# ml-rust/blazr

Hardware: AMD Instinct MI355X
Metric: decode tokens/sec, Llama-3-8B AWQ-INT4 seq=1 on MI355X (and HBM-roofline fraction) (higher is better)
Workload: dtype i4; 1 GPU; llama3-8b-awq greedy decode, batch 1, seq=1, prompt 16 (seed 26), whole step as one hipGraph; N>1 = independent replicas; resident_weight_bytes=5754585088, context_at_end=242

## Files before the change

blazr_amd/csrc/bz_dev.h:

```cpp
#pragma once
#include "bz_internal.h"
#include <math.h>

typedef unsigned int u32x4_t __attribute__((ext_vector_type(4)));
typedef float f32x4_t __attribute__((ext_vector_type(4)));
__device__ __forceinline__ uint4 ldnt(const uint4* p) {
  const u32x4_t v = __builtin_nontemporal_load((const u32x4_t*)p);
  return make_uint4(v.x, v.y, v.z, v.w);
}
__device__ __forceinline__ float4 ldnt(const float4* p) {
  const f32x4_t v = __builtin_nontemporal_load((const f32x4_t*)p);
  return make_float4(v.x, v.y, v.z, v.w);
}

__device__ __forceinline__ float bf16_round(float x) {
  unsigned u = __float_as_uint(x);
  if ((u & 0x7fffffffu) > 0x7f800000u) return x;
  u += 0x7fffu + ((u >> 16) & 1u);
  return __uint_as_float(u & 0xffff0000u);
}
__device__ __forceinline__ float round_act(float x, int act) {
  if (act == BZ_F16) return f16_round(x);
  if (act == BZ_BF16) return bf16_round(x);
  return x;
}
__device__ __forceinline__ double fix_scale(int act) { return act == BZ_F16 ? 17592186044416.0 : (act == BZ_BF16 ? 1099511627776.0 : 4294967296.0); }
__device__ __forceinline__ double fix_inv(int act) { return act == BZ_F16 ? 5.6843418860808015e-14 : (act == BZ_BF16 ? 9.094947017729282e-13 : 2.3283064365386963e-10); }
__device__ __forceinline__ float fix2f(long long a, int act) {
  const unsigned long long m = a < 0 ? (unsigned long long)(-a) : (unsigned long long)a;
  const double d = fma((double)(unsigned)(m >> 32), 4294967296.0, (double)(unsigned)(m & 0xffffffffull)) * fix_inv(act);
  const float r = (float)d;
  return a < 0 ? -r : r;
}
__device__ __forceinline__ long long f2fix(float p, int act) { return __float2ll_rn(p * (float)fix_scale(act)); }
__device__ __forceinline__ float vsrc_get(const VSrc& s, int i, int act) {
  if (s.fix) return round_act(fix2f(((const long long*)s.p)[i], act), act);
  return ((const float*)s.p)[i];
}
__device__ __forceinline__ float silu_f(float x) { return div_rn(x, 1.0f + bz_expf(-x)); }


#define XQ_NP 8
#define XQ_NM 6
struct OpOr { __device__ __forceinline__ static int f(int a, int b) { return a | b; } };
__device__ __forceinline__ int xq_pack_low(int s6, int s7, int flag) { return (s6 & 0xFFF) | ((s7 & 0xFFF) << 12) | (flag ? (1 << 24) : 0); }
__device__ __forceinline__ bool xq_low(const int4* gpar, int gi) { return __builtin_amdgcn_readfirstlane(gpar[gi + 1].w >> 24) != 0; }

__device__ __forceinline__ void xq_split8(const float (&v)[8], float am, unsigned (&w)[XQ_NP], int (&sp)[XQ_NP], float& cscale) {
  const unsigned eb = (__float_as_uint(am) >> 23) & 255u;
  const bool live = eb >= 32u && eb < 255u;
  const float inv = live ? __uint_as_float((283u - eb) << 23) : 0.f;
  cscale = live ? __uint_as_float((eb - 29u) << 23) : 0.f;
  unsigned code[8];
#pragma unroll
  for (int i = 0; i < 8; i++) code[i] = ((unsigned)(int)rintf(v[i] * inv) + 0x88888888u) ^ 0x88888888u;
  unsigned E[4], O[4];
#pragma unroll
  for (int i = 0; i < 4; i++) {
    E[i] = ((code[i + 4] & 0x0F0F0F0Fu) << 4) | (code[i] & 0x0F0F0F0Fu);
    O[i] = ((code[i] >> 4) & 0x0F0F0F0Fu) | (code[i + 4] & 0xF0F0F0F0u);
  }
#pragma unroll
  for (int k = 0; k < 4; k++) {
    const unsigned sel = 0x0c0c0000u | ((4u + k) << 8) | (unsigned)k;
    const int pe = k == 0 ? 6 : 2 * k - 2, po = k == 0 ? 7 : 2 * k - 1;
    w[pe] = __builtin_amdgcn_perm(E[1], E[0], sel) | (__builtin_amdgcn_perm(E[3], E[2], sel) << 16);
    w[po] = __builtin_amdgcn_perm(O[1], O[0], sel) | (__builtin_amdgcn_perm(O[3], O[2], sel) << 16);
  }
#pragma unroll
  for (int p = 0; p < XQ_NP; p++) sp[p] = __builtin_amdgcn_sdot8((int)w[p], 0x11111111, 0, false);
}
template <int NL>
__device__ __forceinline__ int4 xq_gpar_hi(const unsigned (&w)[XQ_NP], const int (&sp)[XQ_NP]) {
  const int fl = grp_reduce<NL, OpOr>((int)((w[6] | w[7]) != 0u));
  return make_int4(sp[3], sp[4], sp[5], xq_pack_low(sp[6], sp[7], fl));
}

template <int NTH>
__device__ __forceinline__ void quant_x128(const float* xs, int KR, uint4* pl, int4* gpar) {
  unsigned* plw = (unsigned*)pl;
  for (int base = 0; base < KR; base += NTH * 8) {
    const int e0 = base + threadIdx.x * 8;
    const bool on = e0 < KR;
    float v[8];
    if (on) {
      float4 a = *(const float4*)(xs + e0), b = *(const float4*)(xs + e0 + 4);
      v[0] = a.x; v[1] = a.y; v[2] = a.z; v[3] = a.w; v[4] = b.x; v[5] = b.y; v[6] = b.z; v[7] = b.w;
    } else {
#pragma unroll
      for (int i = 0; i < 8; i++) v[i] = 0.f;
    }
    float am = 0.f;
#pragma unroll
    for (int i = 0; i < 8; i++) am = fmaxf(am, fabsf(v[i]));
    am = grp_reduce<16, OpMax>(am);
    unsigned w[XQ_NP]; int sp[XQ_NP]; float cs;
    xq_split8(v, am, w, sp, cs);
#pragma unroll
    for (int p = 0; p < XQ_NP; p++) sp[p] = grp_reduce<16, OpAdd>(sp[p]);
    const int4 g2w = xq_gpar_hi<16>(w, sp);
    if (on) {
      const int word = ((e0 >> 5) * XQ_NP) * 4 + ((e0 >> 3) & 3);
#pragma unroll
      for (int p = 0; p < XQ_NP; p++) plw[word + p * 4] = w[p];
      if ((threadIdx.x & 15) == 0) {
        gpar[2 * (e0 >> 7)] = make_int4(__float_as_int(cs), sp[0], sp[1], sp[2]);
        gpar[2 * (e0 >> 7) + 1] = g2w;
      }
    }
  }
}

__device__ __forceinline__ void quant_x64(const float* a, uint4* pl, int4* gpar) {
  const int t = threadIdx.x;
  if (t >= 64) return;
  const bool on = t < 8;
  float v[8];
#pragma unroll
  for (int i = 0; i < 8; i++) v[i] = on ? a[t * 8 + i] : 0.f;
  float am = 0.f;
#pragma unroll
  for (int i = 0; i < 8; i++) am = fmaxf(am, fabsf(v[i]));
  am = grp_reduce<8, OpMax>(am);
  unsigned w[XQ_NP]; int sp[XQ_NP]; float cs;
  xq_split8(v, am, w, sp, cs);
#pragma unroll
  for (int p = 0; p < XQ_NP; p++) sp[p] = grp_reduce<8, OpAdd>(sp[p]);
  const int4 g2w = xq_gpar_hi<8>(w, sp);
  if (on) {
    unsigned* plw = (unsigned*)pl;
    const int word = ((t >> 2) * XQ_NP) * 4 + (t & 3);
#pragma unroll
    for (int p = 0; p < XQ_NP; p++) plw[word + p * 4] = w[p];
    if (t == 0) {
      gpar[0] = make_int4(__float_as_int(cs), sp[0], sp[1], sp[2]);
      gpar[1] = g2w;
    }
  }
}


__device__ __forceinline__ void q4_chunk(const uint4& w, const uint4* pl8, int (&D)[XQ_NM]) {
  const unsigned W[4] = {w.x, w.y, w.z, w.w};
#pragma unroll
  for (int p = 0; p < XQ_NM; p++) {
    const uint4 P = pl8[p];
    const unsigned X[4] = {P.x, P.y, P.z, P.w};
#pragma unroll
    for (int j = 0; j < 4; j++) D[p] = __builtin_amdgcn_sdot8((int)W[j], (int)X[j], D[p], false);
  }
}
__device__ __forceinline__ void q4_chunk_low(const uint4& w, const uint4* pl8, int (&DL)[2]) {
  const unsigned W[4] = {w.x, w.y, w.z, w.w};
#pragma unroll
  for (int p = 0; p < 2; p++) {
    const uint4 P = pl8[XQ_NM + p];
    const unsigned X[4] = {P.x, P.y, P.z, P.w};
#pragma unroll
    for (int j = 0; j < 4; j++) DL[p] = __builtin_amdgcn_sdot8((int)W[j], (int)X[j], DL[p], false);
  }
}
__device__ __forceinline__ void q4_chunk2(const uint4& wa, const uint4& wb, const uint4* pl8, int (&Da)[XQ_NM], int (&Db)[XQ_NM]) {
  const unsigned Wa[4] = {wa.x, wa.y, wa.z, wa.w}, Wb[4] = {wb.x, wb.y, wb.z, wb.w};
#pragma unroll
  for (int p = 0; p < XQ_NM; p++) {
    const uint4 P = pl8[p];
    const unsigned X[4] = {P.x, P.y, P.z, P.w};
#pragma unroll
    for (int j = 0; j < 4; j++) {
      Da[p] = __builtin_amdgcn_sdot8((int)Wa[j], (int)X[j], Da[p], false);
      Db[p] = __builtin_amdgcn_sdot8((int)Wb[j], (int)X[j], Db[p], false);
    }
  }
}
__device__ __forceinline__ int q4_low(const int (&DL)[2], const int4 g2, int z) {
  const int zz = 8 - z, s6 = (g2.w << 20) >> 20, s7 = (g2.w << 8) >> 20;
  return (DL[0] + zz * s6) + ((DL[1] + zz * s7) << 4);
}
__device__ __forceinline__ double q4_term(const int (&D)[XQ_NM], int lw, const int4 g1, const int4 g2, float s, int z) {
  const int zz = 8 - z;
  const int V0 = D[0] + zz * g1.y, V1 = D[1] + zz * g1.z, V2 = D[2] + zz * g1.w, V3 = D[3] + zz * g2.x, V4 = D[4] + zz * g2.y, V5 = D[5] + zz * g2.z;
  const int lo = V0 + (V1 << 4) + (V2 << 8), hi = V3 + (V4 << 4) + (V5 << 8);
  return (double)(s * __int_as_float(g1.x)) * fma(fma((double)hi, 4096.0, (double)lo), 256.0, (double)lw);
}

template <int OFF, int NCH, int NTOT, bool SB = false>
__device__ __forceinline__ void q4g_consume_at(const uint4 (&w)[NTOT], int co, int gp, const uint4* pl, const int4* gpar, float s, int z, double& y) {
  int D[XQ_NM] = {0, 0, 0, 0, 0, 0};
  if (!xq_low(gpar, gp)) {
#pragma unroll
    for (int c = 0; c < NCH; c++) { q4_chunk(w[OFF + c], pl + (co + c) * XQ_NP, D); if (SB) __builtin_amdgcn_sched_barrier(0); }
    y += q4_term(D, 0, gpar[gp], gpar[gp + 1], s, z);
  } else {
    int DL[2] = {0, 0};
#pragma unroll
    for (int c = 0; c < NCH; c++) { q4_chunk(w[OFF + c], pl + (co + c) * XQ_NP, D); q4_chunk_low(w[OFF + c], pl + (co + c) * XQ_NP, DL); if (SB) __builtin_amdgcn_sched_barrier(0); }
    y += q4_term(D, q4_low(DL, gpar[gp + 1], z), gpar[gp], gpar[gp + 1], s, z);
  }
}
template <int NCH>
__device__ __forceinline__ void q4g_consume_n(const uint4 (&w)[NCH], int co, int gp, const uint4* pl, const int4* gpar, float s, int z, double& y) {
  q4g_consume_at<0, NCH, NCH>(w, co, gp, pl, gpar, s, z, y);
}
__device__ __forceinline__ void q4g_consume(const uint4 (&w)[4], int g, const uint4* pl, const int4* gpar, float s, int z, double& y) {
  q4g_consume_at<0, 4, 4>(w, g * 4, 2 * g, pl, gpar, s, z, y);
}
template <int OA, int OB, bool SB, int NA, int NB>
__device__ __forceinline__ void q4g_consume2_x(const uint4 (&wa)[NA], const uint4 (&wb)[NB], int g, const uint4* pl, const int4* gpar, float sa, int za, float sb, int zb,
                                               double& ya, double& yb) {
  int Da[XQ_NM] = {0, 0, 0, 0, 0, 0}, Db[XQ_NM] = {0, 0, 0, 0, 0, 0};
  const int4 g1 = gpar[2 * g], g2 = gpar[2 * g + 1];
  if (!xq_low(gpar, 2 * g)) {
#pragma unroll
    for (int c = 0; c < 4; c++) { q4_chunk2(wa[OA + c], wb[OB + c], pl + (g * 4 + c) * XQ_NP, Da, Db); if (SB) __builtin_amdgcn_sched_barrier(0); }
    ya += q4_term(Da, 0, g1, g2, sa, za);
    yb += q4_term(Db, 0, g1, g2, sb, zb);
  } else {
    int La[2] = {0, 0}, Lb[2] = {0, 0};
#pragma unroll
    for (int c = 0; c < 4; c++) {
      q4_chunk2(wa[OA + c], wb[OB + c], pl + (g * 4 + c) * XQ_NP, Da, Db);
      q4_chunk_low(wa[OA + c], pl + (g * 4 + c) * XQ_NP, La); q4_chunk_low(wb[OB + c], pl + (g * 4 + c) * XQ_NP, Lb);
      if (SB) __builtin_amdgcn_sched_barrier(0);
    }
    ya += q4_term(Da, q4_low(La, g2, za), g1, g2, sa, za);
    yb += q4_term(Db, q4_low(Lb, g2, zb), g1, g2, sb, zb);
  }
}
template <int OFF, int NTOT>
__device__ __forceinline__ void q4g_consume2_at(const uint4 (&wa)[NTOT], const uint4 (&wb)[NTOT], int g, const uint4* pl, const int4* gpar, float sa, int za, float sb, int zb,
                                                double& ya, double& yb) {
  q4g_consume2_x<OFF, OFF, false>(wa, wb, g, pl, gpar, sa, za, sb, zb, ya, yb);
}
template <int OA, int OB, int NTOT, bool SB = false>
__device__ __forceinline__ void q4g_consume2_ab(const uint4 (&w)[NTOT], int g, const uint4* pl, const int4* gpar, float sa, int za, float sb, int zb, double& ya, double& yb) {
  q4g_consume2_x<OA, OB, SB>(w, w, g, pl, gpar, sa, za, sb, zb, ya, yb);
}

__device__ __forceinline__ long long d2fix(double p, int act) { return __double2ll_rn(p * fix_scale(act)); }

template <int ACT> __device__ __forceinline__ float round_t(float x) {
  if (ACT == BZ_F16) return f16_round(x);
  if (ACT == BZ_BF16) return bf16_round(x);
  return x;
}
#define DPP_ROR4 0x124
#define DPP_ROR8 0x128


__device__ __forceinline__ void lds_wait_count(volatile unsigned* cnt, unsigned n) {
  while (*cnt < n) __builtin_amdgcn_s_sleep(1);
  asm volatile("" ::: "memory");
}

__device__ __forceinline__ size_t kv_row_off(const KvView& kv, int layer, int kvh, int p) {
  if (kv.paged) {
    const int blk = kv.block_table[p / kv.bs];
    return (size_t)layer * kv.layer_stride + (((size_t)blk * kv.n_kv + kvh) * kv.bs + (p % kv.bs)) * kv.hd;
  }
  return (size_t)layer * kv.layer_stride + ((size_t)kvh * kv.cap + p) * kv.hd;
}
__device__ __forceinline__ size_t kv_slot_off(const KvView& kv, int layer, int kvh, int slot) {
  const int blk = slot / kv.bs, o = slot % kv.bs;
  return (size_t)layer * kv.layer_stride + (((size_t)blk * kv.n_kv + kvh) * kv.bs + o) * kv.hd;
}
// ... 38 lines not shown
```

blazr_amd/csrc/bz_kernels.hip:

```cpp
#include "bz_internal.h"
#include "bz_dev.h"
#include "bz_ggml.h"
#include <math.h>

#include <hip/hip_ext.h>

static thread_local BzTimingSink* g_sink = nullptr;
void bzk_set_timing_sink(BzTimingSink* s) { g_sink = s; }
BzTimingSink* bzk_timing_sink() { return g_sink; }

__device__ __forceinline__ float block_sum256(float v, float* red) {
  v = wave_sum(v);
  if ((threadIdx.x & 63) == 0) red[threadIdx.x >> 6] = v;
  __syncthreads();
  float t = (red[0] + red[1]) + (red[2] + red[3]);
  __syncthreads();
  return t;
}

template <int NTH>
__device__ __forceinline__ void zero_duty(long long* zb, int zn) {
  if (zb)
    for (int i = blockIdx.x * NTH + threadIdx.x; i < zn; i += gridDim.x * NTH) zb[i] = 0;
}
// ... 2761 lines not shown
#pragma unroll
    for (int i = 0; i < NV; i++) {
      if (KVDT == BZ_F32) {
        const float4 v = *(const float4*)(src + i * 4);
        raw[i] = make_uint4(__float_as_uint(v.x), __float_as_uint(v.y), __float_as_uint(v.z), __float_as_uint(v.w));
      } else {
        unsigned u[4];
#pragma unroll
        for (int j = 0; j < 4; j++) {
          const float x0 = src[i * 8 + 2 * j], x1 = src[i * 8 + 2 * j + 1];
          if (KVDT == BZ_F16) u[j] = (unsigned)__half_as_ushort(f16_cvt(x0)) | ((unsigned)__half_as_ushort(f16_cvt(x1)) << 16);
          else u[j] = (__float_as_uint(bf16_round(x0)) >> 16) | (__float_as_uint(bf16_round(x1)) & 0xffff0000u);
        }
        raw[i] = make_uint4(u[0], u[1], u[2], u[3]);
      }
    }
  }
  __device__ __forceinline__ float get(int e) const {
    if (KVDT == BZ_F32) {
      const uint4 v = raw[e >> 2];
      const unsigned u = (e & 3) == 0 ? v.x : ((e & 3) == 1 ? v.y : ((e & 3) == 2 ? v.z : v.w));
      return __uint_as_float(u);
    }
    const uint4 v = raw[e >> 3];
    const int w = (e >> 1) & 3;
    const unsigned u = w == 0 ? v.x : (w == 1 ? v.y : (w == 2 ? v.z : v.w));
    if (KVDT == BZ_F16) return __half2float(__ushort_as_half((unsigned short)((e & 1) ? (u >> 16) : (u & 0xffffu))));
    return __uint_as_float((e & 1) ? (u & 0xffff0000u) : (u << 16));
  }
};

template <int HD, int KVDT>
__global__ __launch_bounds__(256) void k_attn_decode(AttnArgs a) {
  extern __shared__ __attribute__((aligned(16))) char smem[];
  constexpr int half = HD / 2;
  constexpr int LDR = HD + 4;
  const int rep = a.nq / a.nkv;
  float* qs = (float*)smem;
  float* knew = qs + HD;
  float* vnew = knew + HD;
  float* wred = vnew + HD;
  float* ored = wred + 8;
  const int hq = blockIdx.x, kvh = hq / rep;
  const int tid = threadIdx.x, wave = __builtin_amdgcn_readfirstlane(tid >> 6), lane = tid & 63;
  const int pos = a.pos[0];
  const int len = a.q_only ? pos : pos + 1;
  const int ncache = pos;
  const KvView& kv = a.kv;
  zero_duty<256>(a.zero_buf, a.zero_n);

  if (!a.q_only) {
    const float* cr = a.cos_t + (size_t)pos * half;
    const float* sr = a.sin_t + (size_t)pos * half;
    for (int idx = tid; idx < 2 * half; idx += 256) {
      const int hh = idx / half, i = idx % half;
      const int base = hh == 0 ? hq * HD : a.nq * HD + kvh * HD;
      const int ia = a.interleaved ? 2 * i : i, ib = a.interleaved ? 2 * i + 1 : i + half;
      const float x0 = vsrc_get(a.qkv, base + ia, a.act), x1 = vsrc_get(a.qkv, base + ib, a.act);
      const float c = cr[i], s = sr[i];
      const float y0 = round_act(rope_lo(x0, x1, c, s), a.act), y1 = round_act(rope_hi(x0, x1, c, s), a.act);
      if (hh == 0) { qs[ia] = y0; qs[ib] = y1; }
      else { knew[ia] = y0; knew[ib] = y1; }
    }
    for (int i = tid; i < HD; i += 256) vnew[i] = vsrc_get(a.qkv, a.nq * HD + a.nkv * HD + kvh * HD + i, a.act);
    __syncthreads();
    if (hq % rep == 0) {
      size_t woff;
      if (kv.paged) woff = kv_slot_off(kv, a.layer, kvh, kv.slot ? kv.slot[0] : (kv.block_table[pos / kv.bs] * kv.bs + pos % kv.bs));
      else woff = kv_row_off(kv, a.layer, kvh, pos);
      for (int i = tid; i < HD; i += 256) { kv_st(kv.k, woff + i, kv.dtype, knew[i]); kv_st(kv.v, woff + i, kv.dtype, vnew[i]); }
    }
  } else {
    for (int i = tid; i < HD; i += 256) qs[i] = ((const float*)a.qkv.p)[hq * HD + i];
    __syncthreads();
  }

  const float scale = div_rn(1.0f, sqrt_rn((float)HD));
  float m = -INFINITY, l = 0.f;
  float o[HD];
#pragma unroll
  for (int i = 0; i < HD; i++) o[i] = 0.f;
  for (int p = tid; p < len; p += 256) {
    KvRow<HD, KVDT> kr, vr;
    const size_t ro = p < ncache ? kv_row_off(kv, a.layer, kvh, p) : 0;
    if (p < ncache) kr.load(kv.k, ro); else kr.from_f32(knew);
    if (KVDT != BZ_F32) { if (p < ncache) vr.load(kv.v, ro); else vr.from_f32(vnew); }
    float d = 0.f;
#pragma unroll
    for (int i = 0; i < HD; i += 4) {
      const float4 qa = *(const float4*)(qs + i);
      d += kr.get(i) * qa.x + kr.get(i + 1) * qa.y + kr.get(i + 2) * qa.z + kr.get(i + 3) * qa.w;
    }
    if (KVDT == BZ_F32) { if (p < ncache) vr.load(kv.v, ro); else vr.from_f32(vnew); }
    const float s = d * scale;
    if (m == -INFINITY) {
      m = s; l = 1.f;
#pragma unroll
      for (int i = 0; i < HD; i++) o[i] = vr.get(i);
    } else {
      const float mn = fmaxf(m, s);
      const float alpha = bz_expf(m - mn), e = bz_expf(s - mn);
      l = l * alpha + e;
      m = mn;
#pragma unroll
      for (int i = 0; i < HD; i++) o[i] = o[i] * alpha + e * vr.get(i);
    }
  }
  const float wm = wave_max(m);
  if (lane == 0) wred[wave] = wm;
  __syncthreads();
  const float M = fmaxf(fmaxf(wred[0], wred[1]), fmaxf(wred[2], wred[3]));
  const float w = (m == -INFINITY) ? 0.f : bz_expf(m - M);
  const float ws = wave_sum(l * w);
  if (lane == 0) wred[4 + wave] = ws;
  const int nrows = min(len, 256);
  if (tid < nrows) {
#pragma unroll
    for (int i = 0; i < HD; i += 4) *(float4*)(ored + tid * LDR + i) = make_float4(o[i] * w, o[i + 1] * w, o[i + 2] * w, o[i + 3] * w);
  }
  __syncthreads();
  const float inv = div_rn(1.0f, (wred[4] + wred[5]) + (wred[6] + wred[7]));
  constexpr int PH = 256 / HD;
  const int col = tid % HD, ph = tid / HD;
  float acc = 0.f;
  for (int r = ph; r < nrows; r += PH) acc += ored[r * LDR + col];
  __syncthreads();
  ored[ph * LDR + col] = acc;
  __syncthreads();
  if (tid < HD) {
    float t = 0.f;
#pragma unroll
    for (int q = 0; q < PH; q++) t += ored[q * LDR + tid];
    a.out[(size_t)hq * HD + tid] = round_act(t * inv, a.act);
  }
}


template <int KVDT, int FUSE, int TPW, int NW, int PAGED, int HD = 128>
__global__ __launch_bounds__(NW * 64) void k_attn2(AttnArgs a, const uint4* __restrict__ W, const __half* __restrict__ S,
                                               const unsigned char* __restrict__ Z, const float* __restrict__ bias, int CS, long long* acc) {
  static_assert(HD == 128 || (HD == 64 && FUSE != 1), "head_dim 128, or 64 without the int4 o_proj");
  constexpr int half = HD / 2, NPC = HD / 8, RPL = 64 / NPC, PW = 256 / NW, NL = PW / RPL, OW = NW > 8 ? 8 : NW, NTH = NW * 64;
  asm volatile("" :: "s"(a.zero_buf), "s"(a.zero_n), "s"(a.kv.k), "s"(a.kv.v), "s"(a.kv.cap), "s"(a.kv.layer_stride), "s"(a.layer), "s"(a.act),
               "s"(a.interleaved), "s"(a.rope_cur), "s"(a.qkv.p), "s"(a.qkv.fix), "s"(a.nq), "s"(a.nkv), "s"(a.q_only), "s"(a.pos), "s"(W), "s"(S),
               "s"(Z), "s"(bias), "s"(CS), "s"(acc), "s"(a.out), "s"(a.kv.bs), "s"(a.kv.n_kv));
  extern __shared__ __attribute__((aligned(16))) char smem[];
  unsigned* q2 = (unsigned*)smem;
  unsigned* k2 = q2 + 64;
  unsigned* v2 = k2 + 64;
  double* pout = (double*)(v2 + 64);
  double* lred = pout + NW * 128;
  float* wred = (float*)(lred + NW);
  float* outh = wred + 2 * NW;
  uint4* xpl = (uint4*)(outh + 128);
  int4* gpar = (int4*)(xpl + 4 * XQ_NP);
  const int rep = a.nq / a.nkv;
  const int hq = FUSE ? blockIdx.x / CS : blockIdx.x, cs = FUSE ? blockIdx.x % CS : 0, kvh = hq / rep;
  const int tid = threadIdx.x, wave = __builtin_amdgcn_readfirstlane(tid >> 6), lane = tid & 63;
  const int piece = lane % NPC, rsub = lane / NPC;
  const KvView& kv = a.kv;
  const int pos_v = a.pos[0];
  const int slot_v = PAGED ? *(kv.slot ? kv.slot : a.pos) : 0;
  const int fixq = a.q_only ? 0 : a.qkv.fix;
  int i0, i1;
  {
    const int hh = tid / half, i = tid % half;
    const int base = hh == 0 ? hq * HD : a.nq * HD + kvh * HD;
    const int ia = a.interleaved ? 2 * i : i, ib = a.interleaved ? 2 * i + 1 : i + half;
    const int vb = a.nq * HD + a.nkv * HD + kvh * HD + 2 * i;
    i0 = hh < 2 ? base + ia : vb; i1 = hh < 2 ? base + ib : vb + 1;
    if (a.q_only) { i0 = hq * HD + 2 * i; i1 = i0 + 1; }
    if (hh > 2) { i0 = 0; i1 = 0; }
  }
  unsigned r0l, r0h, r1l, r1h;
  vsrc_issue(a.qkv.p, fixq, i0, r0l, r0h);
  vsrc_issue(a.qkv.p, fixq, i1, r1l, r1h);
  const float* rc = a.q_only ? (const float*)a.qkv.p : a.rope_cur;
  const float pc = rc[tid % half], ps = rc[half + tid % half];
  if (a.zero_buf) {
    const int nblk = FUSE ? a.nq * CS : a.nq;
    for (int i = blockIdx.x * NTH + tid; i < a.zero_n; i += nblk * NTH) a.zero_buf[i] = 0;
  }
  uint4 Wb[FUSE == 1 ? TPW : 1][4];
  const int t0 = (cs * OW + wave % OW) * TPW;
  constexpr int DLD = FUSE == 2 ? TPW : 1;
  uint4 Wd[DLD];
  const int nd0 = (cs * NW + wave) * DLD * RPL;
  if (FUSE == 2) {
    const int K = a.nq * HD;
    const unsigned short* wd = (const unsigned short*)W;
#pragma unroll
    for (int t = 0; t < DLD; t++) Wd[t] = ldnt((const uint4*)(wd + (size_t)(nd0 + t * RPL + rsub) * K + hq * HD + piece * 8));
  }
  if (FUSE == 1) {
    const int K = a.nq * HD;
#pragma unroll
    for (int t = 0; t < TPW; t++) {
      const uint4* wp = W + ((size_t)(t0 + t) * (K >> 5) + hq * 4) * 64 + lane;
#pragma unroll
      for (int c = 0; c < 4; c++) Wb[t][c] = ldnt(wp + c * 64);
    }
  }
  __builtin_amdgcn_sched_barrier(0);
  const int pos = __builtin_amdgcn_readfirstlane(pos_v);
  const int pmax = pos > 0 ? pos - 1 : 0;
  const int len = a.q_only ? pos : pos + 1;
  const unsigned short* kb0 = (const unsigned short*)kv.k + (size_t)a.layer * kv.layer_stride;
  const unsigned short* vb0 = (const unsigned short*)kv.v + (size_t)a.layer * kv.layer_stride;
  uint4 kr[NL], vr[NL];
#pragma unroll
  for (int i = 0; i < NL; i++) { kr[i] = make_uint4(0, 0, 0, 0); vr[i] = make_uint4(0, 0, 0, 0); }
#define ATT_ROW(i) (((i) * NW + wave) * RPL + rsub)
#define ATT_LIVE(c0_, i) ((c0_) + ((i) * NW + wave) * RPL < len)
  if (wave * RPL < len) {
    if (!PAGED) {
      const unsigned short* kb = kb0 + (size_t)kvh * kv.cap * HD;
      const unsigned short* vb = vb0 + (size_t)kvh * kv.cap * HD;
#pragma unroll
      for (int i = 0; i < NL; i++) {
        if (ATT_LIVE(0, i)) {
          const unsigned off = (unsigned)min(ATT_ROW(i), pmax) * HD + piece * 8;
          kr[i] = *(const uint4*)(kb + off);
          vr[i] = *(const uint4*)(vb + off);
        }
      }
    } else {
      int blk[NL];
#pragma unroll
      for (int i = 0; i < NL; i++) blk[i] = ATT_LIVE(0, i) ? kv.block_table[min(ATT_ROW(i), pmax) / kv.bs] : 0;
#pragma unroll
      for (int i = 0; i < NL; i++) {
        if (ATT_LIVE(0, i)) {
          const int pp = min(ATT_ROW(i), pmax);
          const size_t off = (((size_t)blk[i] * kv.n_kv + kvh) * kv.bs + (pp % kv.bs)) * HD + piece * 8;
          kr[i] = *(const uint4*)(kb0 + off);
          vr[i] = *(const uint4*)(vb0 + off);
        }
      }
    }
  }
  const float px0 = vsrc_finish(fixq, r0l, r0h, a.act), px1 = vsrc_finish(fixq, r1l, r1h, a.act);
  if (!a.q_only) {
    if (tid < 2 * half) {
      const int hh = tid / half, i = tid % half;
      const int ia = a.interleaved ? 2 * i : i, ib = a.interleaved ? 2 * i + 1 : i + half;
      const float y0 = round_act(rope_lo(px0, px1, pc, ps), a.act), y1 = round_act(rope_hi(px0, px1, pc, ps), a.act);
      unsigned short* dst = (unsigned short*)(hh == 0 ? q2 : k2);
      const unsigned p0 = pack2<KVDT>(y0, y1);
      dst[ia] = (unsigned short)(p0 & 0xffffu);
      dst[ib] = (unsigned short)(p0 >> 16);
    } else if (tid < 3 * half) {
      v2[tid - 2 * half] = pack2<KVDT>(px0, px1);
    }
    __syncthreads();
    if (hq % rep == 0 && cs == 0 && tid < half) {
      size_t woff;
      if (PAGED) woff = kv_slot_off(kv, a.layer, kvh, kv.slot ? slot_v : (kv.block_table[pos / kv.bs] * kv.bs + pos % kv.bs));
      else woff = kv_row_off_t<0>(kv, a.layer, kvh, pos);
      ((unsigned*)((unsigned short*)kv.k + woff))[tid] = k2[tid];
      ((unsigned*)((unsigned short*)kv.v + woff))[tid] = v2[tid];
    }
  } else {
    if (tid < half) q2[tid] = pack2<KVDT>(px0, px1);
    __syncthreads();
  }

  const float scale = div_rn(1.0f, sqrt_rn((float)HD));
  const uint4 qq = ((const uint4*)q2)[piece];
  float qf[8];
  unpack2<KVDT>(qq.x, qf[0], qf[1]); unpack2<KVDT>(qq.y, qf[2], qf[3]); unpack2<KVDT>(qq.z, qf[4], qf[5]); unpack2<KVDT>(qq.w, qf[6], qf[7]);
  const bool single = len <= 256;
  float sc_[NL];
  float Mw = -INFINITY;
#define ATT_SCORES(c0_)                                                                                                    \
  _Pragma("unroll") for (int i = 0; i < NL; i++) {                                                                         \
    if (!ATT_LIVE(c0_, i)) { sc_[i] = -INFINITY; continue; }                                                               \
    const int p = (c0_) + ATT_ROW(i);                                                                                      \
    uint4 kk = kr[i];                                                                                                      \
    if (!a.q_only && p == pos) { kk = ((const uint4*)k2)[piece]; vr[i] = ((const uint4*)v2)[piece]; }                      \
    float kf[8];                                                                                                           \
    unpack2<KVDT>(kk.x, kf[0], kf[1]); unpack2<KVDT>(kk.y, kf[2], kf[3]); unpack2<KVDT>(kk.z, kf[4], kf[5]); unpack2<KVDT>(kk.w, kf[6], kf[7]); \
    double d = 0.0;                                                                                                        \
    _Pragma("unroll") for (int e = 0; e < 8; e++) d = fma((double)kf[e], (double)qf[e], d);                                \
    d = grp_sum_d<NPC>(d);                                                                                                 \
    sc_[i] = (p < len) ? (float)d * scale : -INFINITY;                                                                     \
  }
  for (int c0 = 0; c0 < len; c0 += 256) {
    const bool won = c0 + wave * RPL < len;
    if (!won) continue;
    if (c0 > 0) {
#pragma unroll
      for (int i = 0; i < NL; i++)
        if (ATT_LIVE(c0, i)) kr[i] = *(const uint4*)(kb0 + kv_row_off_t<PAGED>(kv, 0, kvh, min(c0 + ATT_ROW(i), pmax)) + piece * 8);
    }
    ATT_SCORES(c0)
#pragma unroll
    for (int i = 0; i < NL; i++) Mw = fmaxf(Mw, sc_[i]);
  }
  Mw = wave_max(Mw);
  if (lane == 0) wred[wave] = Mw;
  __syncthreads();
  float Mall = wred[0];
#pragma unroll
  for (int w = 1; w < NW; w++) Mall = fmaxf(Mall, wred[w]);
  double accv[8] = {0.0, 0.0, 0.0, 0.0, 0.0, 0.0, 0.0, 0.0};
  double lsum = 0.0;
  for (int c0 = 0; c0 < len; c0 += 256) {
    const bool won = c0 + wave * RPL < len;
    if (!won) continue;
    if (!single) {
#pragma unroll
      for (int i = 0; i < NL; i++) {
        if (ATT_LIVE(c0, i)) {
          const size_t off = kv_row_off_t<PAGED>(kv, 0, kvh, min(c0 + ATT_ROW(i), pmax)) + piece * 8;
          kr[i] = *(const uint4*)(kb0 + off);
          vr[i] = *(const uint4*)(vb0 + off);
        }
      }
      ATT_SCORES(c0)
    }
#pragma unroll
    for (int i = 0; i < NL; i++) {
      if (!ATT_LIVE(c0, i)) continue;
      const float e = (sc_[i] == -INFINITY) ? 0.f : bz_expf(sc_[i] - Mall);
      const double ed = (double)e;
      lsum += ed;
      float v[8];
      unpack2<KVDT>(vr[i].x, v[0], v[1]); unpack2<KVDT>(vr[i].y, v[2], v[3]);
      unpack2<KVDT>(vr[i].z, v[4], v[5]); unpack2<KVDT>(vr[i].w, v[6], v[7]);
#pragma unroll
      for (int q = 0; q < 8; q++) accv[q] = fma(ed, (double)v[q], accv[q]);
    }
  }
#undef ATT_SCORES
#undef ATT_LIVE
#undef ATT_ROW
  if (NPC == 8) lsum += dpp_get<DPP_ROR8>(lsum);
  lsum = xrow32_d(xrow16_d(lsum));
#pragma unroll
  for (int q = 0; q < 8; q++) {
    if (NPC == 8) accv[q] += dpp_get<DPP_ROR8>(accv[q]);
    accv[q] = xrow32_d(xrow16_d(accv[q]));
  }
  if (lane < NPC) {
#pragma unroll
    for (int q = 0; q < 8; q++) pout[wave * HD + piece * 8 + q] = accv[q];
  }
  if (lane == 0) lred[wave] = lsum;
  __syncthreads();
  float Orun = 0.f, Lrun = 1.f;
  if (tid < HD) {
    double oc = 0.0, Lc = 0.0;
#pragma unroll
    for (int w = 0; w < NW; w++) { oc += pout[w * HD + tid]; Lc += lred[w]; }
    Orun = (float)oc; Lrun = (float)Lc;
  }
  if (!FUSE) {
    if (tid < HD) a.out[(size_t)hq * HD + tid] = round_act(div_rn(Orun, Lrun), a.act);
    return;
  }
  if (tid < HD) outh[tid] = round_act(div_rn(Orun, Lrun), a.act);
  if (FUSE == 2) {
    __syncthreads();
    const float4 oa = *(const float4*)(outh + piece * 8), ob = *(const float4*)(outh + piece * 8 + 4);
    const float of8[8] = {oa.x, oa.y, oa.z, oa.w, ob.x, ob.y, ob.z, ob.w};
#pragma unroll
    for (int t = 0; t < DLD; t++) {
      float w8[8];
      unpack2<KVDT>(Wd[t].x, w8[0], w8[1]); unpack2<KVDT>(Wd[t].y, w8[2], w8[3]); unpack2<KVDT>(Wd[t].z, w8[4], w8[5]); unpack2<KVDT>(Wd[t].w, w8[6], w8[7]);
      double d = 0.0;
#pragma unroll
      for (int e = 0; e < 8; e++) d += (double)__fmul_rn(w8[e], of8[e]);
      d = grp_sum_d<NPC>(d);
      const int n = nd0 + t * RPL + rsub;
      if (piece == 0) {
        if (bias != nullptr && hq == 0) d += (double)bias[n];
        atomicAdd((unsigned long long*)(acc + n), (unsigned long long)d2fix(d, a.act));
      }
    }
    return;
  }
  float sc[FUSE == 1 ? TPW : 1]; int zp[FUSE == 1 ? TPW : 1];
  {
    const int G = (a.nq * HD) >> 7;
#pragma unroll
    for (int t = 0; t < (FUSE == 1 ? TPW : 1); t++) {
      sc[t] = __half2float(S[((size_t)(t0 + t) * G + hq) * 64 + lane]);
      zp[t] = Z[((size_t)(t0 + t) * G + hq) * 64 + lane];
    }
  }
  __syncthreads();
  quant_x128<NW * 64>(outh, HD, xpl, gpar);
  __syncthreads();
#pragma unroll
  for (int t = 0; t < (FUSE == 1 ? TPW : 1); t++) {
    double y = 0.0;
    q4g_consume(Wb[t], 0, xpl, gpar, sc[t], zp[t], y);
    const int n = (t0 + t) * 64 + lane;
    if (bias != nullptr && hq == 0) y += (double)bias[n];
    if (wave < OW) atomicAdd((unsigned long long*)(acc + n), (unsigned long long)d2fix(y, a.act));
  }
}


template <int PAGED, int FUSE = 0>
__global__ __launch_bounds__(512) void k_attn2f(AttnArgs a, const uint4* __restrict__ Wq, const uint4* __restrict__ Hd, const float* __restrict__ bias, int CS, long long* acc) {
  constexpr int HD = 128, half = 64, NW = 8, PW = 256 / NW, NL = PW / 4, NTH = NW * 64;
  __shared__ __attribute__((aligned(16))) float qf[HD], kf[HD], vf[HD];
  __shared__ float wred[2 * NW];
  __shared__ __attribute__((aligned(16))) float pout[NW * 128];
  __shared__ __attribute__((aligned(16))) float outh[FUSE ? HD : 4];
  __shared__ __attribute__((aligned(16))) unsigned xh[FUSE ? 32 : 4], xm[FUSE ? 32 : 4], xl[FUSE ? 32 : 4];
  __shared__ int4 cpar[FUSE ? 8 : 1];
  asm volatile("" :: "s"(a.zero_buf), "s"(a.zero_n), "s"(a.kv.k), "s"(a.kv.v), "s"(a.kv.cap), "s"(a.kv.layer_stride), "s"(a.layer), "s"(a.act),
               "s"(a.interleaved), "s"(a.rope_cur), "s"(a.qkv.p), "s"(a.qkv.fix), "s"(a.nq), "s"(a.nkv), "s"(a.q_only), "s"(a.pos), "s"(a.out),
               "s"(a.kv.bs), "s"(a.kv.n_kv), "s"(Wq), "s"(Hd), "s"(bias), "s"(CS), "s"(acc));
  const int rep = a.nq / a.nkv;
  const int hq = FUSE ? blockIdx.x / CS : blockIdx.x, cs = FUSE ? blockIdx.x % CS : 0, kvh = hq / rep;
  const int tid = threadIdx.x, wave = __builtin_amdgcn_readfirstlane(tid >> 6), lane = tid & 63;
  const int piece = lane & 15, rsub = lane >> 4;
  const KvView& kv = a.kv;
  const int pos_v = a.pos[0];
  const int slot_v = PAGED ? *(kv.slot ? kv.slot : a.pos) : 0;
  const int fixq = a.q_only ? 0 : a.qkv.fix;
  int i0, i1;
  {
    const int hh = tid / half, i = tid % half;
    const int base = hh == 0 ? hq * HD : a.nq * HD + kvh * HD;
    const int ia = a.interleaved ? 2 * i : i, ib = a.interleaved ? 2 * i + 1 : i + half;
    const int vb = a.nq * HD + a.nkv * HD + kvh * HD + 2 * i;
    i0 = hh < 2 ? base + ia : vb; i1 = hh < 2 ? base + ib : vb + 1;
    if (a.q_only) { i0 = hq * HD + 2 * i; i1 = i0 + 1; }
    if (hh > 2) { i0 = 0; i1 = 0; }
  }
  unsigned r0l, r0h, r1l, r1h;
  vsrc_issue(a.qkv.p, fixq, i0, r0l, r0h);
  vsrc_issue(a.qkv.p, fixq, i1, r1l, r1h);
  const float* rc = a.q_only ? (const float*)a.qkv.p : a.rope_cur;
  const float pc = rc[tid % half], ps = rc[half + tid % half];
  if (a.zero_buf)
    for (int i = blockIdx.x * NTH + tid; i < a.zero_n; i += (FUSE ? a.nq * CS : a.nq) * NTH) a.zero_buf[i] = 0;
  uint4 Wb[4]; uint4 hdw = make_uint4(0, 0, 0, 0);
  const int t0 = cs * NW + wave;
  if (FUSE) {
    const int K = a.nq * HD;
    const uint4* wp = Wq + ((size_t)t0 * (K >> 5) + hq * 4) * 64 + lane;
#pragma unroll
    for (int c = 0; c < 4; c++) Wb[c] = ldnt(wp + c * 64);
    hdw = Hd[((size_t)t0 * (K >> 8) + (hq >> 1)) * 64 + lane];
  }
  __builtin_amdgcn_sched_barrier(0);
  const int pos = __builtin_amdgcn_readfirstlane(pos_v);
  const int pmax = pos > 0 ? pos - 1 : 0;
  const int len = a.q_only ? pos : pos + 1;
  const float* kb0 = (const float*)kv.k + (size_t)a.layer * kv.layer_stride;
  const float* vb0 = (const float*)kv.v + (size_t)a.layer * kv.layer_stride;
  float4 kr[NL][2], vr[NL][2];
#pragma unroll
  for (int i = 0; i < NL; i++) { kr[i][0] = kr[i][1] = vr[i][0] = vr[i][1] = make_float4(0.f, 0.f, 0.f, 0.f); }
#define ATF_ROW(i) (((i) * NW + wave) * 4 + rsub)
#define ATF_LIVE(c0_, i) ((c0_) + ((i) * NW + wave) * 4 < len)
  if (wave * 4 < len) {
#pragma unroll
    for (int i = 0; i < NL; i++) {
      if (ATF_LIVE(0, i)) {
        const size_t off = kv_row_off_t<PAGED>(kv, 0, kvh, min(ATF_ROW(i), pmax)) + piece * 8;
        kr[i][0] = *(const float4*)(kb0 + off); kr[i][1] = *(const float4*)(kb0 + off + 4);
        vr[i][0] = *(const float4*)(vb0 + off); vr[i][1] = *(const float4*)(vb0 + off + 4);
      }
    }
  }
  const float px0 = vsrc_finish(fixq, r0l, r0h, a.act), px1 = vsrc_finish(fixq, r1l, r1h, a.act);
  if (!a.q_only) {
    if (tid < 2 * half) {
      const int hh = tid / half, i = tid % half;
      const int ia = a.interleaved ? 2 * i : i, ib = a.interleaved ? 2 * i + 1 : i + half;
      float* dst = hh == 0 ? qf : kf;
      dst[ia] = round_act(rope_lo(px0, px1, pc, ps), a.act);
      dst[ib] = round_act(rope_hi(px0, px1, pc, ps), a.act);
    } else if (tid < 2 * half + 64) {
      vf[2 * (tid - 2 * half)] = px0; vf[2 * (tid - 2 * half) + 1] = px1;
    }
    __syncthreads();
    if (hq % rep == 0 && cs == 0 && tid < HD) {
      size_t woff;
      if (PAGED) woff = kv_slot_off(kv, a.layer, kvh, kv.slot ? slot_v : (kv.block_table[pos / kv.bs] * kv.bs + pos % kv.bs));
      else woff = kv_row_off_t<0>(kv, a.layer, kvh, pos);
      ((float*)kv.k)[woff + tid] = kf[tid];
      ((float*)kv.v)[woff + tid] = vf[tid];
    }
  } else {
    if (tid < 64) { qf[2 * tid] = px0; qf[2 * tid + 1] = px1; }
    __syncthreads();
  }
  const float scale = div_rn(1.0f, sqrt_rn((float)HD));
  const float4 qa = *(const float4*)(qf + piece * 8), qb = *(const float4*)(qf + piece * 8 + 4);
  float Mrun = -INFINITY, Lrun = 0.f, Orun = 0.f;
  for (int c0 = 0; c0 < len; c0 += 256) {
    const bool won = c0 + wave * 4 < len;
    if (c0 > 0) {
      __syncthreads();
      if (won) {
#pragma unroll
        for (int i = 0; i < NL; i++) {
          if (ATF_LIVE(c0, i)) {
            const size_t off = kv_row_off_t<PAGED>(kv, 0, kvh, min(c0 + ATF_ROW(i), pmax)) + piece * 8;
            kr[i][0] = *(const float4*)(kb0 + off); kr[i][1] = *(const float4*)(kb0 + off + 4);
            vr[i][0] = *(const float4*)(vb0 + off); vr[i][1] = *(const float4*)(vb0 + off + 4);
          }
        }
      }
    }
    float sc_[NL];
    float mloc = -INFINITY;
    if (won) {
#pragma unroll
      for (int i = 0; i < NL; i++) {
        if (!ATF_LIVE(c0, i)) { sc_[i] = -INFINITY; continue; }
        const int p = c0 + ATF_ROW(i);
        float4 k0 = kr[i][0], k1 = kr[i][1];
        if (!a.q_only && p == pos) {
          k0 = *(const float4*)(kf + piece * 8); k1 = *(const float4*)(kf + piece * 8 + 4);
          vr[i][0] = *(const float4*)(vf + piece * 8); vr[i][1] = *(const float4*)(vf + piece * 8 + 4);
        }
        float d = k0.x * qa.x + k0.y * qa.y + k0.z * qa.z + k0.w * qa.w + k1.x * qb.x + k1.y * qb.y + k1.z * qb.z + k1.w * qb.w;
        d = grp_reduce<16, OpAdd>(d);
        sc_[i] = (p < len) ? d * scale : -INFINITY;
        mloc = fmaxf(mloc, sc_[i]);
      }
      mloc = wave_max(mloc);
    }
    if (lane == 0) wred[wave] = mloc;
    __syncthreads();
    float Mc = wred[0];
#pragma unroll
    for (int w = 1; w < NW; w++) Mc = fmaxf(Mc, wred[w]);
    float accv[8] = {0.f, 0.f, 0.f, 0.f, 0.f, 0.f, 0.f, 0.f};
    float lsum = 0.f;
    if (won) {
#pragma unroll
      for (int i = 0; i < NL; i++) {
        if (!ATF_LIVE(c0, i)) continue;
        const float e = (sc_[i] == -INFINITY) ? 0.f : bz_expf(sc_[i] - Mc);
        lsum += e;
        accv[0] = fmaf(e, vr[i][0].x, accv[0]); accv[1] = fmaf(e, vr[i][0].y, accv[1]); accv[2] = fmaf(e, vr[i][0].z, accv[2]); accv[3] = fmaf(e, vr[i][0].w, accv[3]);
        accv[4] = fmaf(e, vr[i][1].x, accv[4]); accv[5] = fmaf(e, vr[i][1].y, accv[5]); accv[6] = fmaf(e, vr[i][1].z, accv[6]); accv[7] = fmaf(e, vr[i][1].w, accv[7]);
      }
      lsum = xrow32<OpAdd>(xrow16<OpAdd>(lsum));
#pragma unroll
      for (int q = 0; q < 8; q++) accv[q] = xrow32<OpAdd>(xrow16<OpAdd>(accv[q]));
    }
    if (lane < 16) {
      *(float4*)(pout + wave * 128 + piece * 8) = make_float4(accv[0], accv[1], accv[2], accv[3]);
      *(float4*)(pout + wave * 128 + piece * 8 + 4) = make_float4(accv[4], accv[5], accv[6], accv[7]);
    }
    if (lane == 0) wred[NW + wave] = lsum;
    __syncthreads();
    if (tid < 128) {
      float oc = 0.f, Lc = 0.f;
#pragma unroll
      for (int w = 0; w < NW; w += 2) { oc += pout[w * 128 + tid] + pout[(w + 1) * 128 + tid]; Lc += wred[NW + w] + wred[NW + w + 1]; }
      const float Mn = fmaxf(Mrun, Mc);
      const float fa = (Mrun == -INFINITY) ? 0.f : bz_expf(Mrun - Mn), fb = bz_expf(Mc - Mn);
      Orun = Orun * fa + oc * fb;
      Lrun = Lrun * fa + Lc * fb;
      Mrun = Mn;
    }
  }
  if (!FUSE) {
    if (tid < 128) a.out[(size_t)hq * HD + tid] = round_act(div_rn(Orun, Lrun), a.act);
    return;
  }
  if (tid < 128) outh[tid] = round_act(div_rn(Orun, Lrun), a.act);
  __syncthreads();
  quant_x32<GQ_Q4K>(outh, HD, xh, xm, xl, cpar);
  __syncthreads();
  {
    const unsigned hw[4] = {hdw.x, hdw.y, hdw.z, hdw.w};
    const float d = __half2float(__ushort_as_half((unsigned short)(hw[0] & 0xffffu)));
    const float dmin = __half2float(__ushort_as_half((unsigned short)(hw[0] >> 16)));
    float y = 0.f;
    if (hq & 1) {
#pragma unroll
      for (int c = 0; c < 4; c++) y += gq_chunk_q4k(Wb[c], c, 4 + c, hw, d, dmin, (const uint4*)xh, (const uint4*)xm, (const uint4*)xl, cpar);
    } else {
#pragma unroll
      for (int c = 0; c < 4; c++) y += gq_chunk_q4k(Wb[c], c, c, hw, d, dmin, (const uint4*)xh, (const uint4*)xm, (const uint4*)xl, cpar);
    }
    const int n = t0 * 64 + lane;
    if (bias != nullptr && hq == 0) y += bias[n];
    atomicAdd((unsigned long long*)(acc + n), (unsigned long long)f2fix(y, a.act));
  }
}

static size_t attn2_smem(int nw) { return (size_t)(64 * 3 + 2 * nw + 128 + 4 * XQ_NP * 4 + 8) * 4 + (size_t)(nw * 128 + nw) * 8; }

static int attn_oproj_plan(const AttnArgs& a, const LinearDev& L, int& NW) {
  NW = 0;
  if (a.hd != 128 || L.kind != LK_Q4G || L.perm != nullptr || L.K != a.nq * 128 || a.q_only) return 0;
  const int NT = L.N / 64;
  for (int nw = 8; nw >= 4; nw >>= 1) {
    const int ow = nw > 8 ? 8 : nw;
    for (int cs = 8; cs >= 1; cs >>= 1)
      if (NT % (cs * ow) == 0 && NT / (cs * ow) <= 2 && a.nq * cs <= 1024) { NW = nw; return cs; }
  }
  return 0;
}
static int attn2f_oproj_slices(const AttnArgs& a, const LinearDev& L) {
  static const bool off = getenv("BZ_NO_ATTN_F32") != nullptr;
  if (off || a.hd != 128 || a.kv.dtype != BZ_F32 || a.rope_cur == nullptr || a.q_only || L.kind != LK_Q4K || L.K != a.nq * 128 || L.N % 512 || L.K % 256) return 0;
  const int cs = L.N / 512;
  return a.nq * cs <= 2048 ? cs : 0;
}
static int attn_dense_oproj_loads(const AttnArgs& a, const LinearDev& L) {
  static const bool off = getenv("BZ_NO_ATTN2_HD64") != nullptr;
  if (off || L.kind != LK_ROWS || L.wdt != a.kv.dtype || (a.kv.dtype != BZ_F16 && a.kv.dtype != BZ_BF16) || (a.hd != 64 && a.hd != 128) || a.q_only || a.rope_cur == nullptr) return 0;
  if (L.K != a.nq * a.hd || a.nq * 8 > 2048) return 0;
  const int rpl = 512 / a.hd, per_wave = L.N / 64;
  if (L.N % 64 || per_wave % rpl) return 0;
  const int loads = per_wave / rpl;
  return (loads == 1 || loads == 2 || loads == 4) ? loads : 0;
}
int bzk_attn_oproj_slices(const AttnArgs& a, const LinearDev& L) {
  if (a.kv.dtype == BZ_F32) return attn2f_oproj_slices(a, L);
  if (L.kind == LK_ROWS) return attn_dense_oproj_loads(a, L) > 0 ? 8 : 0;
  int nw; return attn_oproj_plan(a, L, nw);
}

int bzk_attn_oproj(hipStream_t s, const AttnArgs& a, const LinearDev& L, long long* acc) {
  if (a.kv.dtype == BZ_F32) {
    const int CS = attn2f_oproj_slices(a, L);
    if (CS <= 0) BZ_FAIL(BZ_E_INVALID, "attn+o_proj fusion (f32 cache) does not apply to this shape");
    if (a.kv.paged) BZ_LAUNCH("attn+o_proj<q4_K>", L.algo_bytes, (k_attn2f<1, 1>), dim3(a.nq * CS), dim3(512), 0, s, a, (const uint4*)L.w, (const uint4*)L.hdr, L.bias, CS, acc);
    else BZ_LAUNCH("attn+o_proj<q4_K>", L.algo_bytes, (k_attn2f<0, 1>), dim3(a.nq * CS), dim3(512), 0, s, a, (const uint4*)L.w, (const uint4*)L.hdr, L.bias, CS, acc);
    BZ_HIP(hipGetLastError());
    return BZ_OK;
  }
  if (L.kind == LK_ROWS) {
    const int DL = attn_dense_oproj_loads(a, L);
    if (DL <= 0) BZ_FAIL(BZ_E_INVALID, "attn+o_proj fusion (dense) does not apply to this shape");
#define LAUNCH_AD(DT, T, PG, HDV) BZ_LAUNCH("attn+o_proj<dense>", L.algo_bytes, (k_attn2<DT, 2, T, 8, PG, HDV>), dim3(a.nq * 8), dim3(512), attn2_smem(8), s, a, \
    (const uint4*)L.w, (const __half*)nullptr, (const unsigned char*)nullptr, L.bias, 8, acc)
#define LAUNCH_AD_P(DT, T, HDV) do { if (a.kv.paged) LAUNCH_AD(DT, T, 1, HDV); else LAUNCH_AD(DT, T, 0, HDV); } while (0)
#define LAUNCH_AD_T(DT, HDV) do { if (DL == 1) LAUNCH_AD_P(DT, 1, HDV); else if (DL == 2) LAUNCH_AD_P(DT, 2, HDV); else LAUNCH_AD_P(DT, 4, HDV); } while (0)
#define LAUNCH_AD_H(DT) do { if (a.hd == 64) LAUNCH_AD_T(DT, 64); else LAUNCH_AD_T(DT, 128); } while (0)
    if (a.kv.dtype == BZ_F16) LAUNCH_AD_H(BZ_F16); else LAUNCH_AD_H(BZ_BF16);
#undef LAUNCH_AD_H
#undef LAUNCH_AD_T
#undef LAUNCH_AD_P
#undef LAUNCH_AD
    BZ_HIP(hipGetLastError());
    return BZ_OK;
  }
  int NW;
  const int CS = attn_oproj_plan(a, L, NW);
  if (CS <= 0) BZ_FAIL(BZ_E_INVALID, "attn+o_proj fusion does not apply to this shape");
  const int TPW = (L.N / 64) / (CS * (NW > 8 ? 8 : NW));
#define LAUNCH_AO(DT, T, W_, PG) BZ_LAUNCH("attn+o_proj", L.algo_bytes, (k_attn2<DT, 1, T, W_, PG>), dim3(a.nq * CS), dim3(W_ * 64), attn2_smem(W_), s, a, \
    (const uint4*)L.w, (const __half*)L.scales, (const unsigned char*)L.zeros, L.bias, CS, acc)
#define LAUNCH_AO_W(DT, T, PG) do { if (NW == 8) LAUNCH_AO(DT, T, 8, PG); else LAUNCH_AO(DT, T, 4, PG); } while (0)
#define LAUNCH_AO_P(DT, T) do { if (a.kv.paged) LAUNCH_AO_W(DT, T, 1); else LAUNCH_AO_W(DT, T, 0); } while (0)
#define LAUNCH_AO_T(DT) do { if (TPW == 1) LAUNCH_AO_P(DT, 1); else LAUNCH_AO_P(DT, 2); } while (0)
  if (a.kv.dtype == BZ_F16) LAUNCH_AO_T(BZ_F16);
  else if (a.kv.dtype == BZ_BF16) LAUNCH_AO_T(BZ_BF16);
  else BZ_FAIL(BZ_E_UNSUPPORTED, "attn+o_proj fusion: f32 KV cache not built");
#undef LAUNCH_AO_P
#undef LAUNCH_AO_W
#undef LAUNCH_AO_T
#undef LAUNCH_AO
  BZ_HIP(hipGetLastError());
  return BZ_OK;
}


#define ATT_PSTRIDE 132
#define ATT_MAX_SPLITS 128

__host__ __device__ __forceinline__ int att_split_len(int len) {
  int spl = 128;
  while ((len + spl - 1) / spl > ATT_MAX_SPLITS) spl *= 2;
  return spl;
}

template <int KVDT, int PAGED, int REP>
__global__ __launch_bounds__(REP == 8 ? 512 : 256) void k_attn_split(AttnArgs a, int nsplit, float* __restrict__ ws) {
  constexpr int HD = 128, half = 64, NW = REP == 8 ? 8 : 4, NTH = NW * 64, PW = 128 / NW, NL = PW / 4;
  __shared__ __attribute__((aligned(16))) unsigned q2[REP][64];
  __shared__ __attribute__((aligned(16))) unsigned k2[64], v2[64];
  __shared__ float wred[REP][NW], lred[REP][NW];
  __shared__ __attribute__((aligned(16))) float pout[NW][REP][128];
  asm volatile("" :: "s"(a.kv.k), "s"(a.kv.v), "s"(a.kv.cap), "s"(a.kv.layer_stride), "s"(a.layer), "s"(a.act), "s"(a.interleaved), "s"(a.rope_cur),
               "s"(a.qkv.p), "s"(a.qkv.fix), "s"(a.nq), "s"(a.nkv), "s"(a.pos), "s"(nsplit), "s"(ws), "s"(a.kv.bs), "s"(a.kv.n_kv),
               "s"(a.zero_buf), "s"(a.zero_n));
  const int kvh = blockIdx.x / nsplit, s = blockIdx.x % nsplit;
  const int tid = threadIdx.x, wave = __builtin_amdgcn_readfirstlane(tid >> 6), lane = tid & 63;
  const int piece = lane & 15, rsub = lane >> 4;
  const KvView& kv = a.kv;
  const int pos_v = a.pos[0];
  const int slot_v = PAGED ? *(kv.slot ? kv.slot : a.pos) : 0;
  const int hl = min(tid / half, REP - 1), i = tid % half;
  const int ia = a.interleaved ? 2 * i : i, ib = a.interleaved ? 2 * i + 1 : i + half;
  const int qb = (kvh * REP + hl) * HD;
  unsigned q0l, q0h, q1l, q1h, n0l, n0h, n1l, n1h;
  vsrc_issue(a.qkv.p, a.qkv.fix, qb + ia, q0l, q0h);
  vsrc_issue(a.qkv.p, a.qkv.fix, qb + ib, q1l, q1h);
  {
    const int kb_ = a.nq * HD + kvh * HD, vb_ = a.nq * HD + a.nkv * HD + kvh * HD;
    const bool isk = tid < half;
    vsrc_issue(a.qkv.p, a.qkv.fix, isk ? kb_ + ia : vb_ + 2 * i, n0l, n0h);
    vsrc_issue(a.qkv.p, a.qkv.fix, isk ? kb_ + ib : vb_ + 2 * i + 1, n1l, n1h);
  }
  const float pc = a.rope_cur[i], ps = a.rope_cur[half + i];
  if (a.zero_buf)
    for (int z = blockIdx.x * NTH + tid; z < a.zero_n; z += gridDim.x * NTH) a.zero_buf[z] = 0;
  const int pos = __builtin_amdgcn_readfirstlane(pos_v);
  const int len = pos + 1, pmax = pos > 0 ? pos - 1 : 0;
  const int SPL = att_split_len(len);
  const int p0 = s * SPL;
  if (p0 >= len) return;
  const int p1 = min(p0 + SPL, len);
  const bool owner = p1 == len;
  {
    const float x0 = vsrc_finish(a.qkv.fix, q0l, q0h, a.act), x1 = vsrc_finish(a.qkv.fix, q1l, q1h, a.act);
    const unsigned pk = pack2<KVDT>(round_act(rope_lo(x0, x1, pc, ps), a.act), round_act(rope_hi(x0, x1, pc, ps), a.act));
    ((unsigned short*)q2[hl])[ia] = (unsigned short)(pk & 0xffffu);
    ((unsigned short*)q2[hl])[ib] = (unsigned short)(pk >> 16);
  }
  if (owner && tid < 2 * half) {
    const float x0 = vsrc_finish(a.qkv.fix, n0l, n0h, a.act), x1 = vsrc_finish(a.qkv.fix, n1l, n1h, a.act);
    if (tid < half) {
      const unsigned pk = pack2<KVDT>(round_act(rope_lo(x0, x1, pc, ps), a.act), round_act(rope_hi(x0, x1, pc, ps), a.act));
      ((unsigned short*)k2)[ia] = (unsigned short)(pk & 0xffffu);
      ((unsigned short*)k2)[ib] = (unsigned short)(pk >> 16);
    } else {
      v2[i] = pack2<KVDT>(x0, x1);
    }
  }
  __syncthreads();
  if (owner && tid < 64) {
    size_t woff;
    if (PAGED) woff = kv_slot_off(kv, a.layer, kvh, kv.slot ? slot_v : (kv.block_table[pos / kv.bs] * kv.bs + pos % kv.bs));
    else woff = kv_row_off_t<0>(kv, a.layer, kvh, pos);
    ((unsigned*)((unsigned short*)kv.k + woff))[tid] = k2[tid];
    ((unsigned*)((unsigned short*)kv.v + woff))[tid] = v2[tid];
  }
  const unsigned short* kb0 = (const unsigned short*)kv.k + (size_t)a.layer * kv.layer_stride;
  const unsigned short* vb0 = (const unsigned short*)kv.v + (size_t)a.layer * kv.layer_stride;
  const float scale = div_rn(1.0f, sqrt_rn((float)HD));
// ... 1797 lines not shown
```

Baseline: 679.2 tokens/s.

## Make fused attention o_proj tail per-wave to drop block barriers

In the fused attention plus int4 o_proj kernel, each wave now redundantly combines the partial attention outputs, normalizes them, and quantizes the head vector into its own LDS slice. Only wave-level fences are used, replacing the two block-wide __syncthreads around a shared quantization. The AWQ scale and zero-point loads are hoisted next to the weight prefetch so their latency overlaps the attention work. The cost is more LDS per block and duplicated reduction and quantization work in every wave, which could lower occupancy.

```diff
diff --git a/blazr_amd/csrc/bz_dev.h b/blazr_amd/csrc/bz_dev.h
--- a/blazr_amd/csrc/bz_dev.h
+++ b/blazr_amd/csrc/bz_dev.h
@@ -111,6 +111,36 @@
   }
 }
 
+__device__ __forceinline__ void quant_x128_wave(const float* xs, uint4* pl, int4* gpar, int lane) {
+  const int e0 = (lane & 15) * 8;
+  const float4 a = *(const float4*)(xs + e0), b = *(const float4*)(xs + e0 + 4);
+  const float v[8] = {a.x, a.y, a.z, a.w, b.x, b.y, b.z, b.w};
+  float am = 0.f;
+#pragma unroll
+  for (int i = 0; i < 8; i++) am = fmaxf(am, fabsf(v[i]));
+  am = grp_reduce<16, OpMax>(am);
+  unsigned w[XQ_NP]; int sp[XQ_NP]; float cs;
+  xq_split8(v, am, w, sp, cs);
+#pragma unroll
+  for (int p = 0; p < XQ_NP; p++) sp[p] = grp_reduce<16, OpAdd>(sp[p]);
+  const int4 g2w = xq_gpar_hi<16>(w, sp);
+  if (lane < 16) {
+    unsigned* plw = (unsigned*)pl;
+    const int word = ((e0 >> 5) * XQ_NP) * 4 + ((e0 >> 3) & 3);
+#pragma unroll
+    for (int p = 0; p < XQ_NP; p++) plw[word + p * 4] = w[p];
+    if (lane == 0) {
+      gpar[0] = make_int4(__float_as_int(cs), sp[0], sp[1], sp[2]);
+      gpar[1] = g2w;
+    }
+  }
+}
+__device__ __forceinline__ void wave_lds_sync() {
+  __builtin_amdgcn_fence(__ATOMIC_RELEASE, "wavefront");
+  __builtin_amdgcn_wave_barrier();
+  __builtin_amdgcn_fence(__ATOMIC_ACQUIRE, "wavefront");
+}
+
 __device__ __forceinline__ void quant_x64(const float* a, uint4* pl, int4* gpar) {
   const int t = threadIdx.x;
   if (t >= 64) return;
diff --git a/blazr_amd/csrc/bz_kernels.hip b/blazr_amd/csrc/bz_kernels.hip
--- a/blazr_amd/csrc/bz_kernels.hip
+++ b/blazr_amd/csrc/bz_kernels.hip
@@ -2937,8 +2937,8 @@
   double* lred = pout + NW * 128;
   float* wred = (float*)(lred + NW);
   float* outh = wred + 2 * NW;
-  uint4* xpl = (uint4*)(outh + 128);
-  int4* gpar = (int4*)(xpl + 4 * XQ_NP);
+  uint4* xpl = (uint4*)(outh + NW * 128);
+  int4* gpar = (int4*)(xpl + NW * 4 * XQ_NP);
   const int rep = a.nq / a.nkv;
   const int hq = FUSE ? blockIdx.x / CS : blockIdx.x, cs = FUSE ? blockIdx.x % CS : 0, kvh = hq / rep;
   const int tid = threadIdx.x, wave = __builtin_amdgcn_readfirstlane(tid >> 6), lane = tid & 63;
@@ -2977,6 +2977,7 @@
 #pragma unroll
     for (int t = 0; t < DLD; t++) Wd[t] = ldnt((const uint4*)(wd + (size_t)(nd0 + t * RPL + rsub) * K + hq * HD + piece * 8));
   }
+  unsigned short sraw[FUSE == 1 ? TPW : 1]; int zp[FUSE == 1 ? TPW : 1];
   if (FUSE == 1) {
     const int K = a.nq * HD;
 #pragma unroll
@@ -2984,6 +2985,12 @@
       const uint4* wp = W + ((size_t)(t0 + t) * (K >> 5) + hq * 4) * 64 + lane;
 #pragma unroll
       for (int c = 0; c < 4; c++) Wb[t][c] = ldnt(wp + c * 64);
+    }
+    const int G = K >> 7;
+#pragma unroll
+    for (int t = 0; t < TPW; t++) {
+      sraw[t] = ((const unsigned short*)S)[((size_t)(t0 + t) * G + hq) * 64 + lane];
+      zp[t] = Z[((size_t)(t0 + t) * G + hq) * 64 + lane];
     }
   }
   __builtin_amdgcn_sched_barrier(0);
@@ -3133,6 +3140,31 @@
   }
   if (lane == 0) lred[wave] = lsum;
   __syncthreads();
+  if constexpr (FUSE == 1) {
+    float* oh = outh + wave * HD;
+    uint4* xw = xpl + wave * 4 * XQ_NP;
+    int4* gw = gpar + wave * 2;
+    double o0 = 0.0, o1 = 0.0, Lc = 0.0;
+#pragma unroll
+    for (int w = 0; w < NW; w++) {
+      const double2 pp = *(const double2*)(pout + w * HD + 2 * lane);
+      o0 += pp.x; o1 += pp.y; Lc += lred[w];
+    }
+    const float Lr = (float)Lc;
+    *(float2*)(oh + 2 * lane) = make_float2(round_act(div_rn((float)o0, Lr), a.act), round_act(div_rn((float)o1, Lr), a.act));
+    wave_lds_sync();
+    quant_x128_wave(oh, xw, gw, lane);
+    wave_lds_sync();
+#pragma unroll
+    for (int t = 0; t < TPW; t++) {
+      double y = 0.0;
+      q4g_consume(Wb[t], 0, xw, gw, __half2float(__ushort_as_half(sraw[t])), zp[t], y);
+      const int n = (t0 + t) * 64 + lane;
+      if (bias != nullptr && hq == 0) y += (double)bias[n];
+      if (wave < OW) atomicAdd((unsigned long long*)(acc + n), (unsigned long long)d2fix(y, a.act));
+    }
+    return;
+  }
   float Orun = 0.f, Lrun = 1.f;
   if (tid < HD) {
     double oc = 0.0, Lc = 0.0;
@@ -3163,27 +3195,6 @@
         atomicAdd((unsigned long long*)(acc + n), (unsigned long long)d2fix(d, a.act));
       }
     }
-    return;
-  }
-  float sc[FUSE == 1 ? TPW : 1]; int zp[FUSE == 1 ? TPW : 1];
-  {
-    const int G = (a.nq * HD) >> 7;
-#pragma unroll
-    for (int t = 0; t < (FUSE == 1 ? TPW : 1); t++) {
-      sc[t] = __half2float(S[((size_t)(t0 + t) * G + hq) * 64 + lane]);
-      zp[t] = Z[((size_t)(t0 + t) * G + hq) * 64 + lane];
-    }
-  }
-  __syncthreads();
-  quant_x128<NW * 64>(outh, HD, xpl, gpar);
-  __syncthreads();
-#pragma unroll
-  for (int t = 0; t < (FUSE == 1 ? TPW : 1); t++) {
-    double y = 0.0;
-    q4g_consume(Wb[t], 0, xpl, gpar, sc[t], zp[t], y);
-    const int n = (t0 + t) * 64 + lane;
-    if (bias != nullptr && hq == 0) y += (double)bias[n];
-    if (wave < OW) atomicAdd((unsigned long long*)(acc + n), (unsigned long long)d2fix(y, a.act));
   }
 }
 
@@ -3378,7 +3389,7 @@
   }
 }
 
-static size_t attn2_smem(int nw) { return (size_t)(64 * 3 + 2 * nw + 128 + 4 * XQ_NP * 4 + 8) * 4 + (size_t)(nw * 128 + nw) * 8; }
+static size_t attn2_smem(int nw) { return (size_t)(64 * 3 + 2 * nw + nw * (128 + 4 * XQ_NP * 4 + 8)) * 4 + (size_t)(nw * 128 + nw) * 8; }
 
 static int attn_oproj_plan(const AttnArgs& a, const LinearDev& L, int& NW) {
   NW = 0;
```

After: 674.7 tokens/s, median of 2. About the same (-0.7%).
